# hila-chefer/Transformer-Explainability

Hardware: AMD Instinct MI355X
Metric: relevance maps/sec (ViT-B/16 224^2, batch 64 per GPU, generate_LRP transformer_attribution) (higher is better)
Workload: dtype f32 (3xbf16 split operands, 6 products, fp32 accumulate)

## Files before the change

### include/te_relprop.h

```cpp
#ifndef TE_RELPROP_H
#define TE_RELPROP_H

#include <stddef.h>
#include <stdint.h>

#ifdef __cplusplus
extern "C" {
#endif

typedef void* te_stream_t;
typedef uint16_t te_bf16_t;

enum {
  TE_OK = 0,
  TE_ERR_INVALID_ARG = -1,
  TE_ERR_WORKSPACE = -2,
  TE_ERR_UNSUPPORTED = -3,
  TE_ERR_NO_DEVICE = -4
};

enum { TE_VARIANT_OURS = 0, TE_VARIANT_LRP = 1, TE_IMPL_SIMPLE = 0x100 };

enum { TE_ROLLOUT_NORMALISE = 1, TE_ROLLOUT_CLS_FIXUP = 2, TE_ROLLOUT_ROW0 = 4 };

// ... 65 lines not shown
int te_clone_relprop_scaled_f32(const float* R0, const float* s0, int64_t s0_stride,
                                const float* R1, const float* s1, int64_t s1_stride,
                                const float* R2, const float* s2, int64_t s2_stride,
                                const float* X, float* out, int64_t B, int64_t n, te_stream_t stream);

int te_index_select_relprop_f32(const float* R, const float* X, float* out,
                                int64_t B, int64_t N, int64_t C, int64_t index, te_stream_t stream);

int te_gradcam_headmean_f32(const float* grad, const float* cam, float* out,
                            int64_t B, int64_t H, int64_t N, te_stream_t stream);

size_t te_rollout_workspace_bytes(int64_t L, int64_t B, int64_t N);
size_t te_rollout_row0_workspace_bytes(int64_t B, int64_t N);
int te_rollout_f32(const float* cams, int64_t L, int64_t start_layer, int64_t B, int64_t N,
                   int flags, float* joint, void* ws, size_t ws_bytes, te_stream_t stream);

#define TE_X6_TILE_AUTO 0
#define TE_X6_TILE_128 1
#define TE_X6_TILE_256 2
#define TE_X6_TILE_128x128 3
#define TE_X6_TEST_DROP_HANDOVER 0x200
#define TE_X6_WHOLE_TILES 0x10000
#define TE_X6_TEST_SMALL_GRID 0x4000
#define TE_X6_SLACK_RULE 0x100000
#define TE_X6_STATIC_TILES 0x80000
#define TE_X6_X_PLANES_SIGNED 0x20000
#define TE_X6_TILE_Z_SHIFT 10
#define TE_X6_TILE_C_SHIFT 12
#define TE_X6_PHASE_SPLIT 4
#define TE_X6_PHASE_Z 8
#define TE_X6_PHASE_C 16
#define TE_X6_PHASE_MASK 28
int te_linear_relprop_x6_supported(int64_t T, int64_t in_f, int64_t out_f);
size_t te_linear_relprop_x6_workspace_bytes(int64_t T, int64_t in_f, int64_t out_f);
size_t te_linear_x6_weight_planes_bytes(int64_t in_f, int64_t out_f);
size_t te_linear_x6_planes_bytes(int64_t rows, int64_t K);
int te_linear_x6_prepare_weights_f32(const float* W, int64_t in_f, int64_t out_f, void* planes, size_t planes_bytes,
                                     te_stream_t stream);
int te_linear_x6_split_abs_f32(const float* X, int64_t rows, int64_t K, void* planes, size_t planes_bytes,
                               te_stream_t stream);
int te_linear_relprop_x6_f32(const float* R, const float* r_scale, int64_t r_scale_stride, int64_t rows_per_sample,
                             const float* X, const float* W, const void* w_planes, const void* x_planes,
                             const float* Y, const float* bias, float* out,
                             int64_t T, int64_t in_f, int64_t out_f, int flags, unsigned* status, void* ws,
                             size_t ws_bytes, te_stream_t stream);
int te_linear_relprop_x6_check(const void* ws, int64_t T, int64_t in_f, int64_t out_f, te_stream_t stream);
#define TE_X6_PASS_Z 0
#define TE_X6_PASS_C 1
#define TE_X6_PASS_PRODUCT 2
#define TE_X6_SCHEDULE_STREAM_K 0
#define TE_X6_SCHEDULE_WHOLE_STATIC 1
#define TE_X6_SCHEDULE_WHOLE_CLAIMED 2
int te_linear_x6_schedule(int64_t T, int64_t in_f, int64_t out_f, int pass, int flags, int* schedule);

int te_linear_relprop_x6_general_supported(int64_t T, int64_t in_f, int64_t out_f, int variant);
size_t te_linear_x6_weight_planes_lrp_bytes(int64_t in_f, int64_t out_f);
int te_linear_x6_prepare_weights_lrp_f32(const float* W, int64_t in_f, int64_t out_f, void* planes, size_t planes_bytes,
                                         te_stream_t stream);
size_t te_linear_relprop_x6_general_workspace_bytes(int64_t T, int64_t in_f, int64_t out_f, int variant);
int te_linear_relprop_x6_general_f32(const float* R, const float* r_scale, int64_t r_scale_stride, int64_t rows_per_sample,
                                     const float* X, const float* W, const void* w_planes, const void* w_planes_lrp,
                                     const void* x_abs_planes, const float* Y, const float* bias, float* out,
                                     int64_t T, int64_t in_f, int64_t out_f, float alpha, int variant, int flags,
                                     unsigned* status, void* ws, size_t ws_bytes, te_stream_t stream);

int te_gemm_x6_supported(int64_t T, int64_t K, int64_t M);
size_t te_gemm_x6_workspace_bytes(int64_t T, int64_t K, int64_t M);
int te_linear_x6_split_matrix_f32(const float* A, int64_t rows, int64_t K, int transposed, void* planes,
                                  size_t planes_bytes, te_stream_t stream);
int te_gemm_x6_f32(const float* X, const void* x_planes, const void* w_planes, const float* bias, float* out,
                   int64_t T, int64_t K, int64_t M, int flags, unsigned* status, void* ws, size_t ws_bytes,
                   te_stream_t stream);
int te_linear_x6_split_dual_f32(const float* A, int64_t rows, int64_t K, void* planes, void* planes_abs,
                                size_t planes_bytes, te_stream_t stream);
int te_gelu_backward_x6_planes_f32(const float* dy, const float* x, int64_t rows, int64_t K, void* planes,
                                   size_t planes_bytes, te_stream_t stream);
// ... 300 lines not shown
```

### transformer-explainability_amd/csrc/te_linear_x6.hip

```cpp
#include <algorithm>
#include <cmath>
#include <type_traits>

#include "te_x6.h"

namespace {

constexpr int kRB = 3 * kFrag;
constexpr int kMinFrag = 4;
constexpr int kSpinMillis = 250;
constexpr int kErrWord = 1023;
constexpr int kClaimWord = 1024, kClaimStride = 32;


enum { MODE_Z = 0, MODE_C = 1, MODE_G = 2, MODE_ZI = 3, MODE_Z1 = 4, MODE_CI = 5, MODE_X = 6, MODE_ZS = 7 };

__device__ __forceinline__ float bf16_f32(unsigned b) { return __uint_as_float(b << 16); }

enum { OP_ABS = 0, OP_POS = 1, OP_NEG = 2, OP_ID = 3 };
template <int OP>
__device__ __forceinline__ float apply_op(float x) {
  if constexpr (OP == OP_ID) return x;
  if constexpr (OP == OP_ABS) return __int_as_float(__float_as_int(x) & 0x7fffffff);
  const int b = __float_as_int(x);
// ... 149 lines not shown
}

__device__ __forceinline__ float exact_zi(const float* __restrict__ x, const float* __restrict__ w, int64_t K) {
  float z1 = 0.0f, z2 = 0.0f;
  for (int64_t k = 0; k < K; ++k) {
    const float xv = x[k], wv = w[k];
    z1 = fmaf(fmaxf(xv, 0.0f), fminf(wv, 0.0f), z1);
    z2 = fmaf(fminf(xv, 0.0f), fmaxf(wv, 0.0f), z2);
  }
  return z1 + z2;
}

struct X6Params {
  const unsigned char* A;
  const unsigned char* B;
  int64_t a_group_stride;
  int64_t b_rb_stride;
  int nks;
  unsigned char pad0_[20];
  int ntm, ntn;
  int rows_w;
  int t_fast;
  int whole_tiles;
  int pad1_;
  int ncb;
  int64_t T;
  int in_f, out_f;
  float* partial;
  unsigned* flags;
  unsigned* status;
  long long spin_ticks;
  int drop_handover;
  int small_grid;
  int sched_flags;
  const float* R;
  const float* Y;
  const float* bias;
  const float* X;
  const float* W;
  unsigned char* S;
  const float* rs;
  int64_t rs_stride;
  int rps;
  float* out;
  float scale;
  int accum;
  int x_sign;
// ... 37 lines not shown
  constexpr bool SGN = MODE == MODE_ZS;
  constexpr bool Z_ABS = MODE == MODE_Z || SGN;
  constexpr bool IS_Z = (Z_ABS || MODE == MODE_ZI || MODE == MODE_Z1);
  constexpr bool IS_C = (MODE == MODE_C || MODE == MODE_CI);
  constexpr int G = IS_C ? 6 : 3;
  constexpr int NPA = GEO::NPA, NPB = GEO::NPB;
  constexpr int NP = NPA + NPB;
  static_assert(NPA / 3 == NW, "each wave stages one weight-side block");
  constexpr int PBW = NPB / 3 / NW;
  constexpr int STAGE = NP * kFrag;
  constexpr int GROUPS = NPA / G;
  constexpr int LDS_MAIN = X6Lds<WM, MODE>::MAIN;
  extern __shared__ __attribute__((aligned(16))) unsigned char smem[];

  const int lane = threadIdx.x & 63;
  const int wave = __builtin_amdgcn_readfirstlane(threadIdx.x >> 6);
  const int wm = wave % NWM, wn = wave / NWM;
  const int lane16 = lane * 16;

  const int bid = blockIdx.x, spx = gridDim.x >> 3;
  const int xcd = bid & 7, slot = bid >> 3;
  const int nks = p.nks;
  const int tiles = p.ntm * p.ntn;
  const int tx0 = (int)((int64_t)tiles * xcd / 8), tx1 = (int)((int64_t)tiles * (xcd + 1) / 8);
  const int ntx = tx1 - tx0;
  const int64_t iters = (int64_t)ntx * nks;
  auto cut = [&](int s) -> int64_t {
    int64_t b = iters * s / spx;
    const int r = (int)(b % nks);
    if (p.whole_tiles) return (2 * r < nks) ? b - r : b + (nks - r);
    if (r < kMinFrag) b -= r;
    else if (nks - r < kMinFrag) b += nks - r;
    return b;
  };
  const bool claim = p.whole_tiles == 2;
  unsigned* const claim_ctr = p.flags + kClaimWord + xcd * kClaimStride;
  const int64_t ib = cut(slot), ie = cut(slot + 1);
  if (!claim && ib >= ie) return;
  const int f_tile = (int)(ib / nks), kb = (int)(ib - (int64_t)f_tile * nks);
  const int l_tile = (int)((ie - 1) / nks), ke = (int)(ie - (int64_t)l_tile * nks);
  const bool tail = kb > 0;
  const bool head = (ke < nks) && !(f_tile == l_tile && tail);
  const int full0 = tail ? f_tile + 1 : f_tile, full1 = (ke < nks) ? l_tile - 1 : l_tile;
  const int nseq = (head ? 1 : 0) + (full1 >= full0 ? full1 - full0 + 1 : 0) + (tail ? 1 : 0);

  float* my_part = p.partial + (size_t)bid * GEO::THREADS * GEO::ACC;
  const float* in_part = p.partial + (size_t)(bid - 8) * GEO::THREADS * GEO::ACC;

  for (int seq = 0; claim || seq < nseq; ++seq) {
    int tile, k0, k1;
    if (claim) {
      unsigned* const claimed = reinterpret_cast<unsigned*>(smem + X6Lds<WM, MODE>::MAIN + NW * 512) + 1;
      if (threadIdx.x == 0) *claimed = __hip_atomic_fetch_add(claim_ctr, 1u, __ATOMIC_RELAXED, __HIP_MEMORY_SCOPE_AGENT);
      __syncthreads();
      tile = (int)__builtin_amdgcn_readfirstlane(*claimed);
      if (tile >= ntx) break;
      k0 = 0, k1 = nks;
    } else if (head && seq == 0) {
      tile = l_tile, k0 = 0, k1 = ke;
    } else if (tail && seq == nseq - 1) {
      tile = f_tile, k0 = kb, k1 = (f_tile == l_tile) ? ke : nks;
    } else {
      tile = full0 + seq - (head ? 1 : 0), k0 = 0, k1 = nks;
    }
    tile += tx0;
    int tn, tm;
    if (p.t_fast) {
      tm = tile / p.ntn, tn = tile - tm * p.ntn;
    } else {
      tn = tile / p.ntm, tm = tile - tn * p.ntm;
    }
    const bool dead = (int64_t)tn * GEO::TT + wn * 64 >= p.T;

    const unsigned char* srcA;
    if constexpr (!IS_C)
      srcA = p.A + (int64_t)(tm * GROUPS + wave) * p.a_group_stride + (int64_t)k0 * kRB;
    else
      srcA = p.A + (int64_t)(tm * GROUPS + (wave >> 1)) * p.a_group_stride + (int64_t)k0 * (2 * kRB) + (wave & 1) * kRB;
    const unsigned char* srcB[PBW];
#pragma unroll
    for (int u = 0; u < PBW; ++u) {
      const int cb = min(tn * (GEO::TT / 32) + wave * PBW + u, p.ncb - 1);
      srcB[u] = p.B + (int64_t)cb * p.b_rb_stride + (int64_t)k0 * kRB;
    }
    unsigned char* const ldsA = smem + wave * kRB;
    unsigned char* const ldsB = smem + NPA * kFrag + wave * (PBW * kRB);
    u32x4 breg[SGN ? PBW : 1][3];
    auto stage_a = [&](int stg, int adv) __attribute__((always_inline)) {
      srcA += adv * (G * kFrag);
#pragma unroll
      for (int q = 0; q < 3; ++q) glds16(srcA + q * kFrag + lane16, ldsA + stg * STAGE + q * kFrag);
    };
    auto stage_in = [&](int stg, int adv) __attribute__((always_inline)) {
      srcA += adv * (G * kFrag);
#pragma unroll
      for (int u = 0; u < PBW; ++u) srcB[u] += adv * kRB;
#pragma unroll
      for (int q = 0; q < 3; ++q) glds16(srcA + q * kFrag + lane16, ldsA + stg * STAGE + q * kFrag);
#pragma unroll
      for (int u = 0; u < PBW; ++u)
#pragma unroll
        for (int q = 0; q < 3; ++q) {
          if constexpr (SGN) breg[u][q] = *reinterpret_cast<const u32x4*>(srcB[u] + q * kFrag + lane16);
          else glds16(srcB[u] + q * kFrag + lane16, ldsB + stg * STAGE + (u * 3 + q) * kFrag);
        }
// ... 183 lines not shown
      }
      asm volatile("s_waitcnt vmcnt(0)" ::: "memory");
      __syncthreads();
      if (threadIdx.x == 0) {
        __builtin_amdgcn_fence(__ATOMIC_RELEASE, "agent");
        asm volatile("s_waitcnt vmcnt(0)" ::: "memory");
        if (!p.drop_handover) __hip_atomic_store(flag, 1u, __ATOMIC_RELAXED, __HIP_MEMORY_SCOPE_AGENT);
      }
    };
    if (k1 < nks) {
      publish(my_part, p.flags + bid);
      continue;
    }
    const int tc = lane & 31, h = lane >> 5;
    if (dead) {
      if constexpr (X6Lds<WM, MODE>::STAGED) __builtin_amdgcn_s_barrier();
    } else if constexpr (IS_Z) {
      const int nksS = p.out_f >> 4;
      int64_t tl[2];
      bool live[2], blk[2];
      float f[2];
#pragma unroll
      for (int ni = 0; ni < 2; ++ni) {
        const int cb = tn * (GEO::TT / 32) + wn * 2 + ni;
        const int64_t t = (int64_t)cb * 32 + tc;
        blk[ni] = cb < p.ncb;
        live[ni] = t < p.T;
        tl[ni] = live[ni] ? t : p.T - 1;
        f[ni] = p.rs ? p.rs[(tl[ni] / p.rps) * p.rs_stride] : 1.0f;
      }
      float* const bias_lds = reinterpret_cast<float*>(smem + LDS_MAIN) + wave * 128;
      if (lane < MI * 8) {
        f32x4 bv = {0.0f, 0.0f, 0.0f, 0.0f};
        if (p.bias) bv = *reinterpret_cast<const f32x4*>(p.bias + (tm * (NWM * MI) + wm * MI) * 32 + lane * 4);
        *reinterpret_cast<f32x4*>(bias_lds + lane * 4) = bv;
      }
      if constexpr (X6Lds<WM, MODE>::STAGED) {
        constexpr int NL = (MODE == MODE_Z1) ? 4 : 8;
        __builtin_amdgcn_s_barrier();
        unsigned char* const stg = smem + wave * 16384;
        unsigned rda[4];
#pragma unroll
        for (int g = 0; g < 4; ++g)
          rda[g] = (unsigned)(uintptr_t)stg + tc * 128 + (((2 * g + h) ^ ((tc >> 1) & 7)) << 4);
        const unsigned bia = (unsigned)(uintptr_t)bias_lds + h * 16;
        const int r8 = lane >> 3;
        auto request = [&](int bi, int buf) __attribute__((always_inline)) {
          const int ni = bi / MI, mi = bi % MI;
          const int cb = tn * (GEO::TT / 32) + wn * 2 + ni;
          const int j0 = (tm * (NWM * MI) + wm * MI + mi) * 32;
#pragma unroll
          for (int i = 0; i < 4; ++i) {
            const int row = 8 * i + r8;
            const int64_t t = min((int64_t)cb * 32 + row, p.T - 1);
            const int64_t off = t * p.out_f + j0 + (((lane & 7) ^ ((row >> 1) & 7)) << 2);
            glds16(reinterpret_cast<const unsigned char*>(p.R + off), stg + buf * 8192 + i * 1024);
            if constexpr (MODE != MODE_Z1)
              glds16(reinterpret_cast<const unsigned char*>(p.Y + off), stg + buf * 8192 + 4096 + i * 1024);
          }
        };
        const bool all_blk = blk[0] && blk[1];
        request(0, 0);
        request(1, 1);
#pragma unroll
        for (int bi = 0; bi < 2 * MI; ++bi) {
          const int ni = bi / MI, mi = bi % MI, buf = bi & 1;
          const int cb = tn * (GEO::TT / 32) + wn * 2 + ni;
          const int j0 = (tm * (NWM * MI) + wm * MI + mi) * 32;
          constexpr int kStore = 6;
          const int yl = (bi + 1 < 2 * MI) ? NL : 0, ys = (bi >= 2 ? kStore : 0) + (bi >= 1 ? kStore : 0);
          if (all_blk) asm volatile("s_waitcnt vmcnt(%0)" ::"n"(yl + ys) : "memory");
          else asm volatile("s_waitcnt vmcnt(%0)" ::"n"(yl) : "memory");
          f32x4 r4[4], y4[4], b4[4];
#pragma unroll
          for (int g = 0; g < 4; ++g) {
            asm volatile("ds_read_b128 %0, %1 offset:%2" : "=v"(r4[g]) : "v"(rda[g]), "i"(buf * 8192));
            if constexpr (MODE != MODE_Z1)
              asm volatile("ds_read_b128 %0, %1 offset:%2" : "=v"(y4[g]) : "v"(rda[g]), "i"(buf * 8192 + 4096));
            asm volatile("ds_read_b128 %0, %1 offset:%2" : "=v"(b4[g]) : "v"(bia), "i"((mi * 32 + 8 * g) * 4));
          }
          asm volatile("s_waitcnt lgkmcnt(0)" ::: "memory");
          if (bi + 2 < 2 * MI) request(bi + 2, buf);
          X6_PASS4(r4[0], r4[1], r4[2], r4[3]);
          if constexpr (MODE != MODE_Z1) X6_PASS4(y4[0], y4[1], y4[2], y4[3]);
          X6_PASS4(b4[0], b4[1], b4[2], b4[3]);
          unsigned w[4][3][2];
          unsigned long long any_cancel = 0;
          auto z_of = [&](int g, int c0, f32x2& z2, f32x2& a2) __attribute__((always_inline)) {
            a2 = f32x2{acc[mi][ni][4 * g + c0], acc[mi][ni][4 * g + c0 + 1]};
            if constexpr (Z_ABS)
// ... 84 lines not shown
              }
            }
          }
        }
      } else {
      constexpr int NBUF = (MI == 4) ? 2 : 1;
      f32x4 r4[NBUF][4], y4[NBUF][4];
      auto load_block = [&](int bi, int buf) __attribute__((always_inline)) {
        const int ni = bi / MI, mi = bi % MI;
        const int j0 = (tm * (NWM * MI) + wm * MI + mi) * 32;
        const float* Rrow = p.R + tl[ni] * p.out_f + j0 + 4 * h;
#pragma unroll
        for (int g = 0; g < 4; ++g) r4[buf][g] = *reinterpret_cast<const f32x4*>(Rrow + 8 * g);
        if constexpr (MODE != MODE_Z1) {
          const float* Yrow = p.Y + tl[ni] * p.out_f + j0 + 4 * h;
#pragma unroll
          for (int g = 0; g < 4; ++g) y4[buf][g] = *reinterpret_cast<const f32x4*>(Yrow + 8 * g);
        }
      };
      if constexpr (NBUF == 2) load_block(0, 0);
#pragma unroll
      for (int bi = 0; bi < 2 * MI; ++bi) {
        const int ni = bi / MI, mi = bi % MI, buf = bi % NBUF;
        const int cb = tn * (GEO::TT / 32) + wn * 2 + ni;
        const int j0 = (tm * (NWM * MI) + wm * MI + mi) * 32;
        if constexpr (NBUF == 2) {
          if (bi + 1 < 2 * MI) load_block(bi + 1, buf ^ 1);
        } else {
          load_block(bi, 0);
        }
        unsigned w[4][3][2];
        unsigned bad = 0;
#pragma unroll
        for (int g = 0; g < 4; ++g) {
          const f32x4 b4 = *reinterpret_cast<const f32x4*>(bias_lds + mi * 32 + 8 * g + 4 * h);
          float sv4[4];
#pragma unroll
          for (int c = 0; c < 4; ++c) {
            const float a_abs = acc[mi][ni][4 * g + c];
            float z;
            bool cancel;
            if constexpr (Z_ABS) {
              z = 0.5f * ((y4[buf][g][c] - b4[c]) + a_abs);
              cancel = te_z_cancels(z, a_abs, b4[c]);
            } else if constexpr (MODE == MODE_ZI) {
              z = 0.5f * ((y4[buf][g][c] - b4[c]) - a_abs);
              cancel = te_z_cancels(-z, a_abs, b4[c]);
// ... 46 lines not shown
                float rr = Rrow[jj];
                if (p.rs) rr = rr * f[ni];
                unsigned pl[3];
                split3(te_sd(rr, z), pl);
                unsigned short* d = reinterpret_cast<unsigned short*>(Srow + (int64_t)(jj >> 4) * kRB + ((jj >> 3) & 1) * 512) + (jj & 7);
                d[0] = (unsigned short)pl[0];
                d[kFrag / 2] = (unsigned short)pl[1];
                d[kFrag] = (unsigned short)pl[2];
              }
            }
          }
        }
      }
      }
    } else if constexpr (MODE == MODE_G) {
      float* const bias_lds = reinterpret_cast<float*>(smem + LDS_MAIN) + wave * 128;
      if (lane < MI * 8) {
        f32x4 bv = {0.0f, 0.0f, 0.0f, 0.0f};
        if (p.bias) bv = *reinterpret_cast<const f32x4*>(p.bias + (tm * (NWM * MI) + wm * MI) * 32 + lane * 4);
        *reinterpret_cast<f32x4*>(bias_lds + lane * 4) = bv;
      }
#pragma unroll
      for (int ni = 0; ni < 2; ++ni) {
        const int64_t t = ((int64_t)tn * (GEO::TT / 32) + wn * 2 + ni) * 32 + tc;
        float* orow = p.out + (t < p.T ? t : 0) * p.out_f + (tm * (NWM * MI) + wm * MI) * 32 + 4 * h;
#pragma unroll
        for (int mi = 0; mi < MI; ++mi)
#pragma unroll
          for (int g = 0; g < 4; ++g) {
            const f32x4 b4 = *reinterpret_cast<const f32x4*>(bias_lds + mi * 32 + 8 * g + 4 * h);
            f32x4 o;
#pragma unroll
            for (int c = 0; c < 4; ++c) o[c] = acc[mi][ni][4 * g + c] + b4[c];
            if (t < p.T) *reinterpret_cast<f32x4*>(orow + mi * 32 + 8 * g) = o;
          }
      }
    } else if constexpr (MODE == MODE_X) {
#pragma unroll
      for (int ni = 0; ni < 2; ++ni) {
        const int64_t t = ((int64_t)tn * (GEO::TT / 32) + wn * 2 + ni) * 32 + tc;
        const int64_t off = (t < p.T ? t : 0) * p.out_f + (tm * (NWM * MI) + wm * MI) * 32 + 4 * h;
#pragma unroll
        for (int mi = 0; mi < MI; ++mi) {
          f32x4 xv[4], pv[4];
#pragma unroll
          for (int g = 0; g < 4; ++g) {
            xv[g] = *reinterpret_cast<const f32x4*>(p.X + off + mi * 32 + 8 * g);
            pv[g] = p.accum ? *reinterpret_cast<const f32x4*>(p.out + off + mi * 32 + 8 * g) : f32x4{0.0f, 0.0f, 0.0f, 0.0f};
          }
#pragma unroll
          for (int g = 0; g < 4; ++g) {
            f32x4 o;
#pragma unroll
            for (int c = 0; c < 4; ++c) {
              const float xm = (p.x_sign > 0) ? fmaxf(xv[g][c], 0.0f) : fminf(xv[g][c], 0.0f);
              const float v = p.scale * (xm * acc[mi][ni][4 * g + c]);
              o[c] = p.accum ? pv[g][c] + v : v;
            }
            if (t < p.T) *reinterpret_cast<f32x4*>(p.out + off + mi * 32 + 8 * g) = o;
          }
        }
      }
    } else {
      f32x4 x4[2][MI / 2][4];
      int64_t tt[2];
      bool live[2];
#pragma unroll
      for (int ni = 0; ni < 2; ++ni) {
        const int64_t t = ((int64_t)tn * (GEO::TT / 32) + wn * 2 + ni) * 32 + tc;
        live[ni] = t < p.T;
        tt[ni] = live[ni] ? t : p.T - 1;
#pragma unroll
        for (int il = 0; il < MI / 2; ++il) {
          const float* xr = p.X + tt[ni] * p.in_f + (tm * (NWM * MI / 2) + wm * (MI / 2) + il) * 32 + 4 * h;
#pragma unroll
          for (int g = 0; g < 4; ++g) x4[ni][il][g] = *reinterpret_cast<const f32x4*>(xr + 8 * g);
        }
      }
#pragma unroll
      for (int ni = 0; ni < 2; ++ni)
#pragma unroll
        for (int il = 0; il < MI / 2; ++il) {
          float* orow = p.out + tt[ni] * p.in_f + (tm * (NWM * MI / 2) + wm * (MI / 2) + il) * 32 + 4 * h;
#pragma unroll
          for (int g = 0; g < 4; ++g) {
            f32x4 o;
#pragma unroll
            for (int c = 0; c < 4; ++c) {
              const float xv = x4[ni][il][g][c];
              const float xp = fmaxf(xv, 0.0f), xn = fminf(xv, 0.0f);
              if constexpr (MODE == MODE_C)
                o[c] = p.scale * (xp * acc[2 * il][ni][4 * g + c] + xn * acc[2 * il + 1][ni][4 * g + c]);
// ... 42 lines not shown
  l.s_stride = te_align_up(planes_bytes(T, M), 256);
  l.s = xsets * l.x_stride;
  l.partial = l.s + ssets * l.s_stride;
  l.flags = l.partial + kPartialBytes;
  l.total = l.flags + passes * kFlagBytes;
  return l;
}
inline X6Workspace gemm_workspace(int64_t T, int64_t K, int64_t M) { return x6_workspace(T, K, M, 1, 0, 1); }
inline X6Workspace rule_workspace(int64_t T, int64_t in_f, int64_t out_f) { return x6_workspace(T, in_f, out_f, 1, 1, kRulePasses); }
inline X6Workspace general_workspace(int64_t T, int64_t in_f, int64_t out_f) { return x6_workspace(T, in_f, out_f, 2, 2, kGeneralPasses); }

struct X6WeightPlanes { size_t c, total; };
inline X6WeightPlanes weight_planes(int64_t in_f, int64_t out_f) {
  const size_t c = te_align_up(planes_bytes(out_f, in_f), 256);
  return {c, c + te_align_up(2 * planes_bytes(in_f, out_f), 256)};
}
struct X6WeightPlanesLrp { size_t wn, wpT, wnT, total; };
inline X6WeightPlanesLrp weight_planes_lrp(int64_t in_f, int64_t out_f) {
  const size_t za = te_align_up(planes_bytes(out_f, in_f), 256), ca = te_align_up(planes_bytes(in_f, out_f), 256);
  return {za, 2 * za, 2 * za + ca, 2 * za + 2 * ca};
}

constexpr int kTileMask = TE_X6_TILE_128 | TE_X6_TILE_256 | TE_X6_TILE_128x128;
constexpr int kScheduleFlags = TE_X6_WHOLE_TILES | TE_X6_SLACK_RULE | TE_X6_STATIC_TILES;
constexpr int kProductFlags = kTileMask | kScheduleFlags | TE_X6_TEST_DROP_HANDOVER | TE_X6_TEST_SMALL_GRID;
constexpr int kRuleFlags = kProductFlags | TE_X6_PHASE_MASK | TE_X6_X_PLANES_SIGNED | (kTileMask << TE_X6_TILE_Z_SHIFT) | (kTileMask << TE_X6_TILE_C_SHIFT);

inline int pick_wm(int64_t in_f, int64_t out_f) {
  if (out_f % 256 == 0 && in_f % 128 == 0) return 2;
  if (out_f % 128 == 0 && in_f % 64 == 0) return 1;
  return 0;
}

inline long long spin_ticks_for_current_device() {
  static long long cached[64] = {};
  int dev = 0;
  if (hipGetDevice(&dev) != hipSuccess || dev < 0 || dev >= 64) dev = 0;
  if (cached[dev] == 0) {
    int khz = 0;
    if (hipDeviceGetAttribute(&khz, hipDeviceAttributeWallClockRate, dev) != hipSuccess || khz <= 0) khz = 100000;
    cached[dev] = (long long)khz * kSpinMillis;
  }
  return cached[dev];
}

constexpr double kStepLockShort = 2.27, kStepLockLong = 2.00;
constexpr double kStepSkewShort = 2.60, kStepSkewLong = 2.32;
constexpr int kShortSteps = 48, kLongSteps = 144;
constexpr double kWallMargin = 0.05, kWallMarginPacked = 0.20;
constexpr double kWholeTileSlack = 1.15;
inline double step_time(int nks, double t_short, double t_long) {
  if (nks <= kShortSteps) return t_short;
  if (nks >= kLongSteps) return t_long;
  return t_short + (t_long - t_short) * (nks - kShortSteps) / (kLongSteps - kShortSteps);
}
struct X6Schedule { int ntm, ntn, tiles, spx, whole_tiles; };
inline X6Schedule plan_x6(int wm, int64_t T, int rows_w, int nks, int small_grid, int sched_flags) {
  const int tm = (wm == 2) ? 256 : 128, tt = (wm == 0) ? 128 : 256, geo_max_spx = (wm == 2) ? 32 : (wm == 1) ? 64 : 96;
  X6Schedule s;
  s.ntm = rows_w / tm;
  s.ntn = (int)te_ceil_div(T, tt);
  const int64_t tiles = (int64_t)s.ntm * s.ntn;
  s.tiles = (int)tiles;
  const int max_spx = small_grid ? 2 : geo_max_spx;
  s.spx = (int)std::min<int64_t>(max_spx, std::max<int64_t>(1, te_ceil_div(tiles, 8)));
  const double r = (double)tiles / (8.0 * s.spx), rounds = std::ceil(r);
  bool whole;
  if (sched_flags & TE_X6_WHOLE_TILES) whole = true;
  else if (small_grid) whole = false;
  else if (sched_flags & TE_X6_SLACK_RULE) whole = rounds <= kWholeTileSlack * r;
  else {
    const double margin = ((sched_flags & kTileMask) == TE_X6_TILE_256) ? kWallMarginPacked : kWallMargin;
    whole = rounds * step_time(nks, kStepLockShort, kStepLockLong) <= (1.0 + margin) * r * step_time(nks, kStepSkewShort, kStepSkewLong);
  }
  s.whole_tiles = !whole ? 0 : (sched_flags & TE_X6_STATIC_TILES) ? 1 : 2;
  return s;
}

template <int WM, int MODE>
int launch_x6(const X6Params& p, hipStream_t stream) {
  using GEO = X6Geo<WM>;
  static_assert(GEO::TM == ((WM == 2) ? 256 : 128) && GEO::TT == ((WM == 0) ? 128 : 256), "plan_x6 restates the tile sizes");
  constexpr int lds = X6Lds<WM, MODE>::TOTAL;
  static_assert(lds * (WM == 0 ? 3 : WM == 1 ? 2 : 1) <= 160 * 1024, "LDS of the workgroups of one CU");
  static_assert((size_t)8 * GEO::MAX_SPX * GEO::THREADS * GEO::ACC * 4 <= kPartialBytes && 8 * GEO::MAX_SPX < kErrWord, "workspace");
  auto kern = x6_kernel<WM, MODE>;
  hipError_t e = hipFuncSetAttribute(reinterpret_cast<const void*>(kern), hipFuncAttributeMaxDynamicSharedMemorySize, lds);
  if (e != hipSuccess) return (int)e;
  X6Params q = p;
  const X6Schedule s = plan_x6(WM, p.T, p.rows_w, p.nks, p.small_grid, p.sched_flags);
  static_assert(GEO::MAX_SPX == ((WM == 2) ? 32 : (WM == 1) ? 64 : 96), "plan_x6 restates the grid limit");
  q.ntm = s.ntm;
  q.ntn = s.ntn;
  q.whole_tiles = s.whole_tiles;
  if (!q.status) q.status = q.flags + kErrWord;
  q.spin_ticks = spin_ticks_for_current_device();
  kern<<<dim3(8 * s.spx), dim3(GEO::THREADS), lds, stream>>>(q);
  return TE_OK;
}

template <int MODE>
int launch_x6_mode(int wm, const X6Params& p, hipStream_t stream) {
  if (wm == 2) return launch_x6<2, MODE>(p, stream);
  if (wm == 1) return launch_x6<1, MODE>(p, stream);
  return launch_x6<0, MODE>(p, stream);
}

inline int choose_geo(int wm_max, int64_t T, int64_t rows_w, int pin, int min_tiles_256 = 256, bool small_ok = false) {
  if (pin == TE_X6_TILE_128) return 1;
  if (pin == TE_X6_TILE_256) return wm_max;
  if (pin == TE_X6_TILE_128x128) return 0;
  const int64_t t256 = te_ceil_div(T, 256);
  if (wm_max == 2 && t256 * (rows_w / 256) >= min_tiles_256) return 2;
  if (small_ok && t256 * (rows_w / 128) < 448) return 0;
  return 1;
}
inline int geo_z(int64_t T, int64_t in_f, int64_t out_f, int flags) {
// ... 330 lines not shown
    };
    for (int half = 0; half < (beta != 0.0f ? 2 : 1); ++half) {
      const unsigned char* w1 = half ? Wn : Wp, *w2 = half ? Wp : Wn, *w1T = half ? WnT : WpT, *w2T = half ? WpT : WnT;
      const float sc = half ? -beta : alpha;
      if (half) {
        pass = 0;
        static_assert(kGeneralPasses >= 5, "four passes per half + the region of the per-call error word");
        zero_flag_regions(l.flag_region(ws, 0), 4, stream);
      }
      rc = launch_pass<MODE_Z1>(p, wm_z, w1, Xa, Sa, in_f, out_f, l.flag_region(ws, pass++), stream);
      if (rc != TE_OK) return rc;
      rc = launch_pass<MODE_Z1>(p, wm_z, w2, Xb, Sb, in_f, out_f, l.flag_region(ws, pass++), stream);
      if (rc != TE_OK) return rc;
      rc = x_pass(w1T, Sa, +1, sc, half);
      if (rc != TE_OK) return rc;
      rc = x_pass(w2T, Sb, -1, sc, 1);
      if (rc != TE_OK) return rc;
    }
  }
  TE_RETURN_IF_LAUNCH_FAILED();
  return TE_OK;
}

extern "C" int te_linear_x6_schedule(int64_t T, int64_t in_f, int64_t out_f, int pass, int flags, int* schedule) {
  if (!schedule) return TE_ERR_INVALID_ARG;
  const bool product = pass == TE_X6_PASS_PRODUCT;
  if (pass != TE_X6_PASS_Z && pass != TE_X6_PASS_C && !product) return TE_ERR_INVALID_ARG;
  if ((flags & ~(product ? kProductFlags : kRuleFlags)) != 0) return TE_ERR_INVALID_ARG;
  if (!(product ? te_gemm_x6_supported(T, in_f, out_f) : te_linear_relprop_x6_supported(T, in_f, out_f))) return TE_ERR_UNSUPPORTED;
  const bool c = pass == TE_X6_PASS_C;
  const int wm = product ? geo_product(T, out_f, flags) : c ? geo_c(T, in_f, out_f, flags) : geo_z(T, in_f, out_f, flags);
  const X6Schedule s = plan_x6(wm, T, (int)(c ? 2 * in_f : out_f), (int)((c ? out_f : in_f) / 16),
                               (flags & TE_X6_TEST_SMALL_GRID) ? 1 : 0, flags & (kScheduleFlags | kTileMask));
  schedule[0] = wm == 2 ? TE_X6_TILE_256 : wm == 1 ? TE_X6_TILE_128 : TE_X6_TILE_128x128;
  schedule[1] = s.whole_tiles;
  schedule[2] = 8 * s.spx;
  schedule[3] = s.tiles;
  return TE_OK;
}

extern "C" int te_linear_relprop_x6_check(const void* ws, int64_t T, int64_t in_f, int64_t out_f, te_stream_t stream_) {
  if (!ws || !te_linear_relprop_x6_supported(T, in_f, out_f)) return TE_ERR_INVALID_ARG;
  const X6Workspace l = rule_workspace(T, in_f, out_f);
  unsigned host[kRulePasses][kUsedFlagWords];
  hipError_t e = hipSuccess;
  for (int pass = 0; pass < kRulePasses && e == hipSuccess; ++pass)
    e = hipMemcpyAsync(host[pass], l.flag_region(ws, pass), sizeof(host[pass]), hipMemcpyDeviceToHost, (hipStream_t)stream_);
  if (e == hipSuccess) e = hipStreamSynchronize((hipStream_t)stream_);
  if (e != hipSuccess) return (int)e;
  for (int pass = 0; pass < kRulePasses; ++pass)
    for (int i = 0; i < kUsedFlagWords; ++i)
      if (host[pass][i]) return 1;
  return 0;
}
```

### transformer-explainability_amd/ops.py

```python
from __future__ import annotations

import contextlib
import os
from typing import Optional, Sequence, Tuple

import torch

from . import _lib
from ._lib import (TE_HEADMEAN_CLAMP, TE_HEADMEAN_ROW0, TE_IMPL_SIMPLE, TE_RATIONALE_CLAMP, TE_ROLLOUT_CLS_FIXUP,
                   TE_ROLLOUT_NORMALISE, TE_ROLLOUT_ROW0, TE_VARIANT_LRP, TE_VARIANT_OURS)
from ._lib import (TE_X6_PHASE_C, TE_X6_PHASE_SPLIT, TE_X6_PHASE_Z, TE_X6_TEST_DROP_HANDOVER,
                   TE_X6_TEST_SMALL_GRID, TE_X6_TILE_C_SHIFT, TE_X6_TILE_Z_SHIFT, TE_X6_WHOLE_TILES, TE_X6_X_PLANES_SIGNED)
from ._lib import (TE_X6_PASS_C, TE_X6_PASS_PRODUCT, TE_X6_PASS_Z, TE_X6_SCHEDULE_STREAM_K,
                   TE_X6_SCHEDULE_WHOLE_CLAIMED, TE_X6_SCHEDULE_WHOLE_STATIC, TE_X6_SLACK_RULE, TE_X6_STATIC_TILES)

Tensor = torch.Tensor
_VARIANTS = {"ours": TE_VARIANT_OURS, "lrp": TE_VARIANT_LRP}

FORCE_SIMPLE = False
KERNEL_TIMER = None
_NULL = contextlib.nullcontext()


def _timed(name: str, flops: float = 0.0, nbytes: float = 0.0):
    return _NULL if KERNEL_TIMER is None else KERNEL_TIMER(name, float(flops), float(nbytes))


class Deferred:
    __slots__ = ("t", "scale")

    def __init__(self, t: Tensor, scale: Tensor):
        self.t, self.scale = t, scale

    @property
    def shape(self):
        return self.t.shape

# ... 96 lines not shown
        if not _is_f64(t):
            _prep_bf16(t) if _is_bf16(t) else _prep(t)
        if not _checked_device:
            _lib.require_device()
            _checked_device = True
        self.ctx = torch.cuda.device(t.device)

    def __enter__(self):
        self.ctx.__enter__()
        return _lib.load()

    def __exit__(self, *a):
        return self.ctx.__exit__(*a)


USE_FORWARD_OUTPUT = True
USE_FORWARD_PRODUCTS = True


USE_LINEAR_X6 = os.environ.get("TE_LINEAR_X6", "1") not in ("", "0")
X6_CHECK = False
X6_TILE = 0
X6_FLAGS = int(os.environ.get("TE_X6_FLAGS", "0"), 0)


_x6_status = {}


def _x6_device_index(device) -> int:
    dev = torch.device(device)
    return torch.cuda.current_device() if dev.index is None else dev.index


def x6_status(device) -> Tensor:
    idx = _x6_device_index(device)
    t = _x6_status.get(idx)
    if t is None:
        if torch.cuda.is_current_stream_capturing():
            raise _lib.TeError("the x6 status word must exist before a HIP graph is captured: run the step once eagerly "
                               "(GraphedLRP / GraphedCall warm up before they capture)")
        t = _x6_status[idx] = torch.zeros(4, dtype=torch.int32, device=torch.device("cuda", idx))
    return t


def _x6_failed_words(device=None) -> list:
    keys = list(_x6_status) if device is None else [_x6_device_index(device)]
# ... 227 lines not shown
            if got is not None:
                xs, x_bytes = got[0], 6.0 * T * K
                post_x_abs_planes(keep_abs, X, T, K, got[1] if got[1] is not None else _signed(xs))
        if xs is not None and xs.numel() * xs.element_size() < lib.te_linear_x6_planes_bytes(T, K):
            raise _lib.TeError(f"gemm_x6: the operand planes handed in hold {xs.numel() * xs.element_size()} bytes, "
                               f"[{T}, {K}] needs {lib.te_linear_x6_planes_bytes(T, K)}")
        for_rule = xs is None and keep_abs is not None and rule_takes_abs_planes(T, K, M)
        if for_rule and not X6_SIGNED_PLANES:
            x_bytes += 6.0 * T * K
        with _timed(timer_name, 12.0 * T * K * M, x_bytes + 6.0 * K * M + 4.0 * T * M):
            if for_rule:
                nb = lib.te_linear_x6_planes_bytes(T, K)
                if X6_SIGNED_PLANES:
                    xs = _signed(_ws(nb, Xc))
                    _lib.check(lib.te_linear_x6_split_matrix_f32(_ptr(Xc), T, K, 0, _ptr(xs), nb, _stream(Xc)),
                               "te_linear_x6_split_matrix_f32")
                    post_x_abs_planes(keep_abs, X, T, K, xs)
                else:
                    xs, xa = _ws(nb, Xc), _ws(nb, Xc)
                    _lib.check(lib.te_linear_x6_split_dual_f32(_ptr(Xc), T, K, _ptr(xs), _ptr(xa), nb, _stream(Xc)),
                               "te_linear_x6_split_dual_f32")
                    post_x_abs_planes(keep_abs, X, T, K, xa)
            _lib.check(lib.te_gemm_x6_f32(_ptr(Xc) if Xc is not None else None, _ptr(xs), _ptr(w_planes), _ptr(bc), _ptr(out),
                                          T, K, M, (X6_TILE | X6_FLAGS) & ~0x3c00, _ptr(x6_status(X.device)), _ptr(ws),
                                          ws.numel(), _stream(like)), "te_gemm_x6_f32")
    return out.reshape(*lead, M)


def linear_relprop(R: Tensor, X: Tensor, W: Tensor, alpha: float = 1.0, variant="ours",
                   Y: Optional[Tensor] = None, bias: Optional[Tensor] = None, cache: Optional[dict] = None) -> Tensor:
    if _any_f64(R, X, W):
        return linear_relprop_f64(R, X, W, alpha=alpha, variant=variant)
    if _is_bf16(X) or _is_bf16(W):
        return linear_relprop_bf16(R, X, W, alpha=alpha, variant=variant, cache=cache)
    out_f, in_f = W.shape
    lead = X.shape[:-1]
    R, r_scale = _split_deferred(R)
    Rc, Xc, Wc = _c(R).reshape(-1, out_f), _c(X).reshape(-1, in_f), _c(W)
    T = Xc.shape[0]
    if Rc.shape[0] != T:
        raise _lib.TeError(f"Linear.relprop: R has {Rc.shape[0]} rows, X has {T}")
    out = torch.empty((T, in_f), dtype=torch.float32, device=X.device)
    var = _variant(variant)
    fast_ok = (var == TE_VARIANT_OURS and alpha == 1 and in_f % 4 == 0 and out_f % 4 == 0 and
               all(t.data_ptr() % 16 == 0 for t in (Rc, Xc, Wc)))
    fwd = fast_ok and USE_FORWARD_OUTPUT and Y is not None
    if r_scale is not None and not fwd:
# ... 7 lines not shown
               and all(t.data_ptr() % 16 == 0 for t in (Rc, Xc, Wc))
               and (var_code == TE_VARIANT_LRP or (USE_FORWARD_OUTPUT and Y is not None))
               and bool(_lib.load().te_linear_relprop_x6_general_supported(T, in_f, out_f, var_code)))
    if general:
        Yg = bg = None
        if var_code == TE_VARIANT_OURS:
            Yg = _c(Y.detach()).reshape(-1, out_f)
            bg = None if bias is None else _c(bias.detach())
            general = Yg.shape[0] == T and Yg.data_ptr() % 16 == 0 and (bg is None or bg.data_ptr() % 16 == 0)
    if general:
        wp = x6_weight_planes(W, cache) if var_code == TE_VARIANT_OURS else None
        wpl = x6_weight_planes_lrp(W, cache) if var_code == TE_VARIANT_LRP else None
        xa = take_x_abs_planes(cache, X, T, in_f) if cache is not None and var_code == TE_VARIANT_OURS else None
        if planes_are_signed(xa):
            xa = None
        gemm = 2.0 * T * in_f * out_f
        halves = 2 if alpha != 1 else 1
        units = (18.0 if var_code == TE_VARIANT_OURS else 24.0) * halves
        with _on_device(Xc) as lib, _timed("linear_x6_general", units * gemm,
                                           halves * (6.0 * (2 * T * in_f + 3 * in_f * out_f + 2 * T * out_f) + 16.0 * T * in_f)):
            ws = _ws(lib.te_linear_relprop_x6_general_workspace_bytes(T, in_f, out_f, var_code), Xc)
            _lib.check(lib.te_linear_relprop_x6_general_f32(_ptr(Rc), rs_ptr, rs_stride, rps, _ptr(Xc), _ptr(Wc), _ptr(wp),
                                                            _ptr(wpl), _ptr(xa), _ptr(Yg), _ptr(bg), _ptr(out), T, in_f,
                                                            out_f, float(alpha), var_code, (X6_TILE | X6_FLAGS) & ~0x3c00,
                                                            _ptr(x6_status(Xc.device)), _ptr(ws), ws.numel(), _stream(Xc)),
                       "te_linear_relprop_x6_general_f32")
            if X6_CHECK:
                x6_raise_if_failed(Xc.device)
        return out.reshape(*lead, in_f)
    if fwd:
        Yc = _c(Y.detach()).reshape(-1, out_f)
        bc = None if bias is None else _c(bias.detach())
        if Yc.shape[0] != T:
            raise _lib.TeError(f"Linear.relprop: Y has {Yc.shape[0]} rows, X has {T}")
    if (fwd and USE_LINEAR_X6 and Yc.data_ptr() % 16 == 0 and (bc is None or bc.data_ptr() % 16 == 0)
            and _lib.load().te_linear_relprop_x6_supported(T, in_f, out_f)):
        planes = x6_weight_planes(W, cache)
        xa = take_x_abs_planes(cache, X, T, in_f) if cache is not None else None
        x_signed = TE_X6_X_PLANES_SIGNED if planes_are_signed(xa) else 0
        with _on_device(Xc) as lib:
            ws = _ws(lib.te_linear_relprop_x6_workspace_bytes(T, in_f, out_f), Xc)
            status = x6_status(Xc.device)

            def call(flags):
                _lib.check(lib.te_linear_relprop_x6_f32(_ptr(Rc), rs_ptr, rs_stride, rps, _ptr(Xc), _ptr(Wc), _ptr(planes),
                                                        _ptr(xa), _ptr(Yc), _ptr(bc), _ptr(out), T, in_f, out_f,
                                                        X6_TILE | X6_FLAGS | x_signed | flags, _ptr(status), _ptr(ws), ws.numel(),
                                                        _stream(Xc)),
                           "te_linear_relprop_x6_f32")
            if KERNEL_TIMER is None:
                call(0)
            else:
                gemm = 2.0 * T * in_f * out_f
                if xa is None:
                    with _timed("linear_x6_split", 0.0, 10.0 * T * in_f):
                        call(TE_X6_PHASE_SPLIT)
                else:
                    call(TE_X6_PHASE_SPLIT)
                with _timed("linear_x6_zpass", 6.0 * gemm, 6.0 * (T * in_f + in_f * out_f + T * out_f) + 8.0 * T * out_f):
                    call(TE_X6_PHASE_Z)
                with _timed("linear_x6_cpass", 12.0 * gemm, 6.0 * (T * out_f + 2 * in_f * out_f) + 8.0 * T * in_f):
                    call(TE_X6_PHASE_C)
            if X6_CHECK:
                rc = lib.te_linear_relprop_x6_check(_ptr(ws), T, in_f, out_f, _stream(Xc))
                if rc != 0:
                    status.zero_()
                    raise _lib.TeError(f"te_linear_relprop_x6_f32({T},{in_f},{out_f}): a workgroup waited in vain for the "
                                       f"accumulators of a shared tile (status {rc}); the result is invalid")
                x6_raise_if_failed(Xc.device)
        return out.reshape(*lead, in_f)
    if KERNEL_TIMER is not None and fast_ok:
        with _on_device(Xc) as lib:
            S = torch.empty((T, out_f), dtype=torch.float32, device=X.device)
# ... 1897 lines not shown
```

Before: 1012.

## Add half-width tail tiles to balance whole-tile x6 schedule

Adds a half-tail schedule for the 256-wide x6 GEMM geometry. Full-width tiles cover the complete rounds, and the leftover token columns are split into half-width tiles of four column blocks, so the last partial round fills the grid better. plan_x6 enables this when the tail fits in one grid pass and the timing model favours it. The Python side turns the flag on by default. This adds index arithmetic and new kernel branches, and carries a risk of edge-case errors in the tile mapping.

```diff
diff --git a/include/te_relprop.h b/include/te_relprop.h
--- a/include/te_relprop.h
+++ b/include/te_relprop.h
@@ -111,6 +111,7 @@
 #define TE_X6_TEST_DROP_HANDOVER 0x200
 #define TE_X6_WHOLE_TILES 0x10000
 #define TE_X6_TEST_SMALL_GRID 0x4000
+#define TE_X6_HALF_TAIL 0x400000
 #define TE_X6_SLACK_RULE 0x100000
 #define TE_X6_STATIC_TILES 0x80000
 #define TE_X6_X_PLANES_SIGNED 0x20000
@@ -141,6 +142,8 @@
 #define TE_X6_SCHEDULE_WHOLE_STATIC 1
 #define TE_X6_SCHEDULE_WHOLE_CLAIMED 2
 int te_linear_x6_schedule(int64_t T, int64_t in_f, int64_t out_f, int pass, int flags, int* schedule);
+#define TE_X6_SCHEDULE_WHOLE_HALF_TAIL 3
+int te_linear_x6_schedule_tail(int64_t T, int64_t in_f, int64_t out_f, int pass, int flags, int* tail);
 
 int te_linear_relprop_x6_general_supported(int64_t T, int64_t in_f, int64_t out_f, int variant);
 size_t te_linear_x6_weight_planes_lrp_bytes(int64_t in_f, int64_t out_f);
diff --git a/transformer-explainability_amd/csrc/te_linear_x6.hip b/transformer-explainability_amd/csrc/te_linear_x6.hip
--- a/transformer-explainability_amd/csrc/te_linear_x6.hip
+++ b/transformer-explainability_amd/csrc/te_linear_x6.hip
@@ -195,7 +195,7 @@
   int rows_w;
   int t_fast;
   int whole_tiles;
-  int pad1_;
+  int n_full;
   int ncb;
   int64_t T;
   int in_f, out_f;
@@ -279,8 +279,13 @@
   const int xcd = bid & 7, slot = bid >> 3;
   const int nks = p.nks;
   const int tiles = p.ntm * p.ntn;
-  const int tx0 = (int)((int64_t)tiles * xcd / 8), tx1 = (int)((int64_t)tiles * (xcd + 1) / 8);
-  const int ntx = tx1 - tx0;
+  int n_full = p.ntn;
+  if constexpr (WM == 2) n_full = p.n_full;
+  const int tiles_f = p.ntm * n_full, tiles_h = tiles - tiles_f;
+  const int tx0 = (int)((int64_t)tiles_f * xcd / 8), tx1 = (int)((int64_t)tiles_f * (xcd + 1) / 8);
+  const int hx0 = (int)((int64_t)tiles_h * xcd / 8), hx1 = (int)((int64_t)tiles_h * (xcd + 1) / 8);
+  const int nfx = tx1 - tx0;
+  const int ntx = nfx + (hx1 - hx0);
   const int64_t iters = (int64_t)ntx * nks;
   auto cut = [&](int s) -> int64_t {
     int64_t b = iters * s / spx;
@@ -320,14 +325,19 @@
     } else {
       tile = full0 + seq - (head ? 1 : 0), k0 = 0, k1 = nks;
     }
-    tile += tx0;
+    const bool half = WM == 2 && tile >= nfx;
+    const int cols = half ? p.ntn - n_full : n_full;
+    tile += half ? hx0 - nfx : tx0;
     int tn, tm;
     if (p.t_fast) {
-      tm = tile / p.ntn, tn = tile - tm * p.ntn;
+      tm = tile / cols, tn = tile - tm * cols;
     } else {
       tn = tile / p.ntm, tm = tile - tn * p.ntm;
     }
-    const bool dead = (int64_t)tn * GEO::TT + wn * 64 >= p.T;
+    const int cb0 = half ? 8 * n_full + 4 * tn : tn * (GEO::TT / 32);
+    const int64_t t_end = half ? min(p.T, (int64_t)(cb0 + 4) * 32) : p.T;
+    const int64_t cb0w = half ? (int64_t)cb0 : (int64_t)tn * (GEO::TT / 32);
+    const bool dead = (half ? (int64_t)cb0 * 32 : (int64_t)tn * GEO::TT) + wn * 64 >= t_end;
 
     const unsigned char* srcA;
     if constexpr (!IS_C)
@@ -337,7 +347,7 @@
     const unsigned char* srcB[PBW];
 #pragma unroll
     for (int u = 0; u < PBW; ++u) {
-      const int cb = min(tn * (GEO::TT / 32) + wave * PBW + u, p.ncb - 1);
+      const int cb = min(cb0 + wave * PBW + u, p.ncb - 1);
       srcB[u] = p.B + (int64_t)cb * p.b_rb_stride + (int64_t)k0 * kRB;
     }
     unsigned char* const ldsA = smem + wave * kRB;
@@ -567,7 +577,7 @@
       float f[2];
 #pragma unroll
       for (int ni = 0; ni < 2; ++ni) {
-        const int cb = tn * (GEO::TT / 32) + wn * 2 + ni;
+        const int cb = cb0 + wn * 2 + ni;
         const int64_t t = (int64_t)cb * 32 + tc;
         blk[ni] = cb < p.ncb;
         live[ni] = t < p.T;
@@ -592,7 +602,7 @@
         const int r8 = lane >> 3;
         auto request = [&](int bi, int buf) __attribute__((always_inline)) {
           const int ni = bi / MI, mi = bi % MI;
-          const int cb = tn * (GEO::TT / 32) + wn * 2 + ni;
+          const int cb = cb0 + wn * 2 + ni;
           const int j0 = (tm * (NWM * MI) + wm * MI + mi) * 32;
 #pragma unroll
           for (int i = 0; i < 4; ++i) {
@@ -610,7 +620,7 @@
 #pragma unroll
         for (int bi = 0; bi < 2 * MI; ++bi) {
           const int ni = bi / MI, mi = bi % MI, buf = bi & 1;
-          const int cb = tn * (GEO::TT / 32) + wn * 2 + ni;
+          const int cb = cb0 + wn * 2 + ni;
           const int j0 = (tm * (NWM * MI) + wm * MI + mi) * 32;
           constexpr int kStore = 6;
           const int yl = (bi + 1 < 2 * MI) ? NL : 0, ys = (bi >= 2 ? kStore : 0) + (bi >= 1 ? kStore : 0);
@@ -741,7 +751,7 @@
 #pragma unroll
       for (int bi = 0; bi < 2 * MI; ++bi) {
         const int ni = bi / MI, mi = bi % MI, buf = bi % NBUF;
-        const int cb = tn * (GEO::TT / 32) + wn * 2 + ni;
+        const int cb = cb0 + wn * 2 + ni;
         const int j0 = (tm * (NWM * MI) + wm * MI + mi) * 32;
         if constexpr (NBUF == 2) {
           if (bi + 1 < 2 * MI) load_block(bi + 1, buf ^ 1);
@@ -834,7 +844,7 @@
       }
 #pragma unroll
       for (int ni = 0; ni < 2; ++ni) {
-        const int64_t t = ((int64_t)tn * (GEO::TT / 32) + wn * 2 + ni) * 32 + tc;
+        const int64_t t = (cb0w + wn * 2 + ni) * 32 + tc;
         float* orow = p.out + (t < p.T ? t : 0) * p.out_f + (tm * (NWM * MI) + wm * MI) * 32 + 4 * h;
 #pragma unroll
         for (int mi = 0; mi < MI; ++mi)
@@ -850,7 +860,7 @@
     } else if constexpr (MODE == MODE_X) {
 #pragma unroll
       for (int ni = 0; ni < 2; ++ni) {
-        const int64_t t = ((int64_t)tn * (GEO::TT / 32) + wn * 2 + ni) * 32 + tc;
+        const int64_t t = (cb0w + wn * 2 + ni) * 32 + tc;
         const int64_t off = (t < p.T ? t : 0) * p.out_f + (tm * (NWM * MI) + wm * MI) * 32 + 4 * h;
 #pragma unroll
         for (int mi = 0; mi < MI; ++mi) {
@@ -879,7 +889,7 @@
       bool live[2];
 #pragma unroll
       for (int ni = 0; ni < 2; ++ni) {
-        const int64_t t = ((int64_t)tn * (GEO::TT / 32) + wn * 2 + ni) * 32 + tc;
+        const int64_t t = (cb0w + wn * 2 + ni) * 32 + tc;
         live[ni] = t < p.T;
         tt[ni] = live[ni] ? t : p.T - 1;
 #pragma unroll
@@ -968,7 +978,7 @@
 }
 
 constexpr int kTileMask = TE_X6_TILE_128 | TE_X6_TILE_256 | TE_X6_TILE_128x128;
-constexpr int kScheduleFlags = TE_X6_WHOLE_TILES | TE_X6_SLACK_RULE | TE_X6_STATIC_TILES;
+constexpr int kScheduleFlags = TE_X6_WHOLE_TILES | TE_X6_SLACK_RULE | TE_X6_STATIC_TILES | TE_X6_HALF_TAIL;
 constexpr int kProductFlags = kTileMask | kScheduleFlags | TE_X6_TEST_DROP_HANDOVER | TE_X6_TEST_SMALL_GRID;
 constexpr int kRuleFlags = kProductFlags | TE_X6_PHASE_MASK | TE_X6_X_PLANES_SIGNED | (kTileMask << TE_X6_TILE_Z_SHIFT) | (kTileMask << TE_X6_TILE_C_SHIFT);
 
@@ -1000,7 +1010,8 @@
   if (nks >= kLongSteps) return t_long;
   return t_short + (t_long - t_short) * (nks - kShortSteps) / (kLongSteps - kShortSteps);
 }
-struct X6Schedule { int ntm, ntn, tiles, spx, whole_tiles; };
+constexpr double kHalfTileRatio = 0.60;
+struct X6Schedule { int ntm, ntn, tiles, spx, whole_tiles, n_full, half_cols; };
 inline X6Schedule plan_x6(int wm, int64_t T, int rows_w, int nks, int small_grid, int sched_flags) {
   const int tm = (wm == 2) ? 256 : 128, tt = (wm == 0) ? 128 : 256, geo_max_spx = (wm == 2) ? 32 : (wm == 1) ? 64 : 96;
   X6Schedule s;
@@ -1011,15 +1022,28 @@
   const int max_spx = small_grid ? 2 : geo_max_spx;
   s.spx = (int)std::min<int64_t>(max_spx, std::max<int64_t>(1, te_ceil_div(tiles, 8)));
   const double r = (double)tiles / (8.0 * s.spx), rounds = std::ceil(r);
-  bool whole;
-  if (sched_flags & TE_X6_WHOLE_TILES) whole = true;
+  const int64_t grid = 8 * s.spx, full_rounds = tiles / grid;
+  const int64_t n_full = std::min<int64_t>(s.ntn, full_rounds * grid / s.ntm);
+  const int64_t half_cols = te_ceil_div(te_ceil_div(T, 32) - 8 * n_full, 4);
+  const bool tail_fits = wm == 2 && (sched_flags & TE_X6_HALF_TAIL) && !(sched_flags & TE_X6_STATIC_TILES) && n_full >= 1 &&
+                         half_cols >= 1 && s.ntm * half_cols <= grid;
+  bool whole, tail = false;
+  if (sched_flags & TE_X6_WHOLE_TILES) whole = true, tail = tail_fits;
   else if (small_grid) whole = false;
   else if (sched_flags & TE_X6_SLACK_RULE) whole = rounds <= kWholeTileSlack * r;
   else {
-    const double margin = ((sched_flags & kTileMask) == TE_X6_TILE_256) ? kWallMarginPacked : kWallMargin;
-    whole = rounds * step_time(nks, kStepLockShort, kStepLockLong) <= (1.0 + margin) * r * step_time(nks, kStepSkewShort, kStepSkewLong);
+    const bool packed = (sched_flags & kTileMask) == TE_X6_TILE_256;
+    const double margin = packed ? kWallMarginPacked : kWallMargin;
+    const double t_lock = step_time(nks, kStepLockShort, kStepLockLong), t_skew = step_time(nks, kStepSkewShort, kStepSkewLong);
+    whole = rounds * t_lock <= (1.0 + margin) * r * t_skew;
+    tail = tail_fits && !whole && packed &&
+           ((double)full_rounds + kHalfTileRatio) * t_lock <= (1.0 + margin) * r * t_skew;
+    whole = whole || tail;
   }
   s.whole_tiles = !whole ? 0 : (sched_flags & TE_X6_STATIC_TILES) ? 1 : 2;
+  s.n_full = tail ? (int)n_full : s.ntn;
+  s.half_cols = tail ? (int)half_cols : 0;
+  if (tail) s.ntn = s.n_full + s.half_cols;
   return s;
 }
 
@@ -1039,6 +1063,7 @@
   q.ntm = s.ntm;
   q.ntn = s.ntn;
   q.whole_tiles = s.whole_tiles;
+  q.n_full = s.n_full;
   if (!q.status) q.status = q.flags + kErrWord;
   q.spin_ticks = spin_ticks_for_current_device();
   kern<<<dim3(8 * s.spx), dim3(GEO::THREADS), lds, stream>>>(q);
@@ -1415,20 +1440,43 @@
   return TE_OK;
 }
 
-extern "C" int te_linear_x6_schedule(int64_t T, int64_t in_f, int64_t out_f, int pass, int flags, int* schedule) {
-  if (!schedule) return TE_ERR_INVALID_ARG;
+namespace {
+inline int schedule_of(int64_t T, int64_t in_f, int64_t out_f, int pass, int flags, const int* out, int* wm_out, X6Schedule* s) {
+  if (!out) return TE_ERR_INVALID_ARG;
   const bool product = pass == TE_X6_PASS_PRODUCT;
   if (pass != TE_X6_PASS_Z && pass != TE_X6_PASS_C && !product) return TE_ERR_INVALID_ARG;
   if ((flags & ~(product ? kProductFlags : kRuleFlags)) != 0) return TE_ERR_INVALID_ARG;
   if (!(product ? te_gemm_x6_supported(T, in_f, out_f) : te_linear_relprop_x6_supported(T, in_f, out_f))) return TE_ERR_UNSUPPORTED;
   const bool c = pass == TE_X6_PASS_C;
   const int wm = product ? geo_product(T, out_f, flags) : c ? geo_c(T, in_f, out_f, flags) : geo_z(T, in_f, out_f, flags);
-  const X6Schedule s = plan_x6(wm, T, (int)(c ? 2 * in_f : out_f), (int)((c ? out_f : in_f) / 16),
-                               (flags & TE_X6_TEST_SMALL_GRID) ? 1 : 0, flags & (kScheduleFlags | kTileMask));
+  *wm_out = wm;
+  *s = plan_x6(wm, T, (int)(c ? 2 * in_f : out_f), (int)((c ? out_f : in_f) / 16), (flags & TE_X6_TEST_SMALL_GRID) ? 1 : 0,
+               flags & (kScheduleFlags | kTileMask));
+  return TE_OK;
+}
+}
+
+extern "C" int te_linear_x6_schedule(int64_t T, int64_t in_f, int64_t out_f, int pass, int flags, int* schedule) {
+  int wm;
+  X6Schedule s;
+  const int rc = schedule_of(T, in_f, out_f, pass, flags & ~TE_X6_HALF_TAIL, schedule, &wm, &s);
+  if (rc != TE_OK) return rc;
   schedule[0] = wm == 2 ? TE_X6_TILE_256 : wm == 1 ? TE_X6_TILE_128 : TE_X6_TILE_128x128;
   schedule[1] = s.whole_tiles;
   schedule[2] = 8 * s.spx;
   schedule[3] = s.tiles;
+  return TE_OK;
+}
+
+extern "C" int te_linear_x6_schedule_tail(int64_t T, int64_t in_f, int64_t out_f, int pass, int flags, int* tail) {
+  int wm;
+  X6Schedule s;
+  const int rc = schedule_of(T, in_f, out_f, pass, flags, tail, &wm, &s);
+  if (rc != TE_OK) return rc;
+  tail[0] = s.half_cols ? TE_X6_SCHEDULE_WHOLE_HALF_TAIL : s.whole_tiles;
+  tail[1] = s.ntm * s.n_full;
+  tail[2] = s.ntm * s.half_cols;
+  tail[3] = s.n_full;
   return TE_OK;
 }
 
diff --git a/transformer-explainability_amd/ops.py b/transformer-explainability_amd/ops.py
--- a/transformer-explainability_amd/ops.py
+++ b/transformer-explainability_amd/ops.py
@@ -13,6 +13,7 @@
                    TE_X6_TEST_SMALL_GRID, TE_X6_TILE_C_SHIFT, TE_X6_TILE_Z_SHIFT, TE_X6_WHOLE_TILES, TE_X6_X_PLANES_SIGNED)
 from ._lib import (TE_X6_PASS_C, TE_X6_PASS_PRODUCT, TE_X6_PASS_Z, TE_X6_SCHEDULE_STREAM_K,
                    TE_X6_SCHEDULE_WHOLE_CLAIMED, TE_X6_SCHEDULE_WHOLE_STATIC, TE_X6_SLACK_RULE, TE_X6_STATIC_TILES)
+from ._lib import TE_X6_HALF_TAIL, TE_X6_SCHEDULE_WHOLE_HALF_TAIL
 
 Tensor = torch.Tensor
 _VARIANTS = {"ours": TE_VARIANT_OURS, "lrp": TE_VARIANT_LRP}
@@ -155,6 +156,14 @@
 X6_CHECK = False
 X6_TILE = 0
 X6_FLAGS = int(os.environ.get("TE_X6_FLAGS", "0"), 0)
+X6_HALF_TAIL = {"": False, "0": False, "1": True}.get(os.environ.get("TE_X6_HALF_TAIL", "1"), os.environ.get("TE_X6_HALF_TAIL", "1"))
+
+
+def _x6_flags(kind):
+    if X6_HALF_TAIL not in (True, False, "zg", "c"):
+        raise ValueError(f"ops.X6_HALF_TAIL = {X6_HALF_TAIL!r}: expected True / False / 'zg' / 'c'")
+    on = X6_HALF_TAIL is True or (X6_HALF_TAIL is not False and kind in X6_HALF_TAIL)
+    return X6_TILE | X6_FLAGS | (TE_X6_HALF_TAIL if on else 0)
 
 
 _x6_status = {}
@@ -428,7 +437,7 @@
                                "te_linear_x6_split_dual_f32")
                     post_x_abs_planes(keep_abs, X, T, K, xa)
             _lib.check(lib.te_gemm_x6_f32(_ptr(Xc) if Xc is not None else None, _ptr(xs), _ptr(w_planes), _ptr(bc), _ptr(out),
-                                          T, K, M, (X6_TILE | X6_FLAGS) & ~0x3c00, _ptr(x6_status(X.device)), _ptr(ws),
+                                          T, K, M, _x6_flags("g") & ~0x3c00, _ptr(x6_status(X.device)), _ptr(ws),
                                           ws.numel(), _stream(like)), "te_gemm_x6_f32")
     return out.reshape(*lead, M)
 
@@ -482,7 +491,7 @@
             ws = _ws(lib.te_linear_relprop_x6_general_workspace_bytes(T, in_f, out_f, var_code), Xc)
             _lib.check(lib.te_linear_relprop_x6_general_f32(_ptr(Rc), rs_ptr, rs_stride, rps, _ptr(Xc), _ptr(Wc), _ptr(wp),
                                                             _ptr(wpl), _ptr(xa), _ptr(Yg), _ptr(bg), _ptr(out), T, in_f,
-                                                            out_f, float(alpha), var_code, (X6_TILE | X6_FLAGS) & ~0x3c00,
+                                                            out_f, float(alpha), var_code, _x6_flags("zc") & ~0x3c00,
                                                             _ptr(x6_status(Xc.device)), _ptr(ws), ws.numel(), _stream(Xc)),
                        "te_linear_relprop_x6_general_f32")
             if X6_CHECK:
@@ -503,12 +512,16 @@
             status = x6_status(Xc.device)
 
             def call(flags):
+                kind = {TE_X6_PHASE_Z: "z", TE_X6_PHASE_SPLIT | TE_X6_PHASE_Z: "z", TE_X6_PHASE_C: "c"}.get(flags, "zc")
                 _lib.check(lib.te_linear_relprop_x6_f32(_ptr(Rc), rs_ptr, rs_stride, rps, _ptr(Xc), _ptr(Wc), _ptr(planes),
                                                         _ptr(xa), _ptr(Yc), _ptr(bc), _ptr(out), T, in_f, out_f,
-                                                        X6_TILE | X6_FLAGS | x_signed | flags, _ptr(status), _ptr(ws), ws.numel(),
+                                                        _x6_flags(kind) | x_signed | flags, _ptr(status), _ptr(ws), ws.numel(),
                                                         _stream(Xc)),
                            "te_linear_relprop_x6_f32")
-            if KERNEL_TIMER is None:
+            if KERNEL_TIMER is None and X6_HALF_TAIL in ("zg", "c"):
+                call(TE_X6_PHASE_SPLIT | TE_X6_PHASE_Z)
+                call(TE_X6_PHASE_C)
+            elif KERNEL_TIMER is None:
                 call(0)
             else:
                 gemm = 2.0 * T * in_f * out_f
```

Result: no change. 1017 (median of 6 runs) (+0.5%).
